# neeharperi/FutureDet

Measured on AMD Instinct MI355X. Metric: sweeps/sec end-to-end (300k pts, 10-sweep voxel), higher is better.
Workload: dtype f32

## Files before the change

futuredet_amd/csrc/fd_common.h:

```cpp
#pragma once
#include <hip/hip_runtime.h>
#include <stdint.h>
#include <stdio.h>

#include <atomic>

#include "../../include/futuredet_hip.h"

namespace fd {

void set_error(const char *fmt, ...);
int spconv_f32_compact_dispatch(const float *in, const void *wp, const float *bias, const float *residual, int relu, const int *nbr,
                                int64_t nbr_stride, int K, int64_t n_in_bound, int n_out, const int *n_out_dev, int cin, int cout, float *out,
                                const int *ranges, int n_ranges, hipStream_t stream);

size_t spconv_bf16_win_weight_bytes(int K, int cin, int cout);
void spconv_bf16_win_pack(const float *w, int K, int cin, int cout, uint16_t (*tobf)(float), uint16_t *dst);
int spconv_bf16_win_dispatch(const void *in, const void *wp_win, const float *bias, const void *residual, int relu, const int *nbr, int64_t nbr_stride, int K,
                             int64_t n_in_bound, int n_out, const int *n_out_dev, int64_t n_expected, int cin, int cout, void *out, hipStream_t stream);
int spconv_bf16_ws_dispatch(const void *in, const void *wp, const float *bias, const void *residual, int relu, const int *nbr, int64_t nbr_stride, int K,
                            int64_t n_in_bound, int n_out, const int *n_out_dev, int64_t n_expected, int cin, int cout, void *out, hipStream_t stream);

int wino_pc_launch(const float *x, const void *wp, const float *bias, float *y, int B, int H, int W, int cin, int cout, int relu, int cout_total,
                   int co_off, hipStream_t stream);

int spconv_f32_res16_dispatch(const float *in, const void *wp, const float *bias, const float *residual, int relu, const int *nbr, int64_t nbr_stride, int K,
                              int64_t n_in_bound, int n_out, const int *n_out_dev, int64_t n_expected, int cin, int cout, float *out, hipStream_t stream);

int spconv_f32_c32_dispatch(const float *in, const void *wp, const float *bias, const float *residual, int relu, const int *nbr,
                            int64_t nbr_stride, int K, int64_t n_in_bound, int n_out, const int *n_out_dev, int cin, int cout, float *out,
                            const int *ranges, int n_ranges, hipStream_t stream);

__device__ __forceinline__ int device_count(int capacity, const int *count_dev) {
    if (!count_dev) return capacity;
    const int n = *count_dev;
    return n < capacity ? (n > 0 ? n : 0) : capacity;
}

inline int check_launch(const char *what) {
    hipError_t e = hipGetLastError();
    if (e != hipSuccess) {
        set_error("%s: %s", what, hipGetErrorString(e));
        return FD_ELAUNCH;
    }
    return FD_OK;
}

#define FD_REQUIRE(cond, ...)           \
    do {                                \
        if (!(cond)) {                  \
            fd::set_error(__VA_ARGS__); \
            return FD_EINVAL;           \
        }                               \
    } while (0)

inline hipStream_t as_stream(fd_stream_t s) { return reinterpret_cast<hipStream_t>(s); }

int fill_words(void *p, uint32_t value, size_t n_words, hipStream_t stream);
int fill_words3(void *p0, uint32_t v0, size_t n0, void *p1, uint32_t v1, size_t n1, void *p2, uint32_t v2, size_t n2, hipStream_t stream);

constexpr int kMaxDevices = 64;
int current_device();
int device_cu_count();
bool ensure_dynamic_lds(const void *kernel, size_t bytes, std::atomic<uint64_t> &done);
enum TuneKey { kTuneSpconvRG = 0, kTuneSpconvV1, kTuneSpconvBf16V1, kTuneV2Depth, kTuneV2TM, kTuneV2LdsPad, kTuneConvNT, kTuneV2RangesPerCU, kTuneV2Uniform, kTuneV2RowCost, kTuneSpconvC32, kTuneBf16GP, kTuneBf16RG, kTuneBf16Depth, kTuneBf16NW, kTuneStrict, kTuneBf16Win, kTuneF32ResRG, kTuneConvStrip, kTuneF32ResNW, kTuneCount };
int tuning(TuneKey key);

inline size_t align_up(size_t v, size_t a) { return (v + a - 1) / a * a; }

struct IndexGeom {
    int B, D, H, W, Ht, Wt;
    __host__ __device__ int64_t num_cols() const { return (int64_t)B * Ht * Wt * 64; }
};
__host__ __device__ inline IndexGeom make_geom(int B, int D, int H, int W) {
    IndexGeom g;
    g.B = B; g.D = D; g.H = H; g.W = W;
    g.Ht = (H + 7) >> 3; g.Wt = (W + 7) >> 3;
    return g;
}
__host__ __device__ inline int64_t col_of(const IndexGeom &g, int b, int y, int x) {
    return ((((int64_t)b * g.Ht + (y >> 3)) * g.Wt + (x >> 3)) << 6) + ((y & 7) << 3) + (x & 7);
}
__device__ inline void col_to_byx(const IndexGeom &g, int64_t col, int &b, int &y, int &x) {
    int in = (int)(col & 63);
    int64_t t = col >> 6;
    int tx = (int)(t % g.Wt);
    t /= g.Wt;
    int ty = (int)(t % g.Ht);
    b = (int)(t / g.Ht);
    y = ty * 8 + (in >> 3);
    x = tx * 8 + (in & 7);
}

__device__ inline unsigned xcd_swizzle(unsigned bid, unsigned nblocks) {
    const unsigned nx = 8;
    unsigned per = nblocks / nx, rem = nblocks % nx;
    unsigned xcd = bid % nx, loc = bid / nx;
    unsigned start = xcd * per + (xcd < rem ? xcd : rem);
    return start + loc;
}

}
```

futuredet_amd/csrc/fd_conv2d_wino.hip:

```cpp
#include "fd_common.h"

#ifndef FD_WINO_OCC16
#define FD_WINO_OCC16 3
#endif

namespace {

#ifdef FD_V2_TRACE
__device__ unsigned long long *g_wtrace;
#define FD_WT(var) const unsigned long long var = __builtin_readcyclecounter()
#define FD_WDECL unsigned long long wacc[8] = {0, 0, 0, 0, 0, 0, 0, 0}
#define FD_WADD(i, v) wacc[i] += (v)
#define FD_WFLUSH                                                                                              \
    do {                                                                                                       \
        if (threadIdx.x == 0 && g_wtrace)                                                                      \
            for (int i_ = 0; i_ < 8; ++i_) g_wtrace[(size_t)(blockIdx.x + blockIdx.y * gridDim.x) * 8 + i_] = wacc[i_]; \
    } while (0)
#else
#define FD_WT(var)
#define FD_WDECL
#define FD_WADD(i, v)
#define FD_WFLUSH
#endif

typedef float f32x4 __attribute__((ext_vector_type(4)));

struct WinoParams {
    int B, H, W, Cin, Cout_pad, Cout_real, cout_total, co_off, relu;
    int tiles_x, tiles_y;
};

__device__ __forceinline__ float4 f4add(float4 a, float4 b) { return make_float4(a.x + b.x, a.y + b.y, a.z + b.z, a.w + b.w); }
__device__ __forceinline__ float4 f4sub(float4 a, float4 b) { return make_float4(a.x - b.x, a.y - b.y, a.z - b.z, a.w - b.w); }

template <int TY, int TX, int NBW>
__global__ void __launch_bounds__(256, (TY * TX * NBW <= 16) ? FD_WINO_OCC16 : (TY * TX * NBW <= 32) ? 2 : 1) conv2d_wino_f32(const float *__restrict__ x, const float4 *__restrict__ wp, const float *__restrict__ bias,
                                                       float *__restrict__ y, WinoParams p) {
    constexpr int NTILE = TY * TX, NTB = NTILE / 16;
    static_assert(NTILE % 16 == 0, "tiles per workgroup must fill whole MFMA blocks");
    constexpr int PH = 2 * TY + 2, PW = 2 * TX + 2, PP = PH * PW;
    constexpr int NCHUNK = PP * 4, NLOAD = (NCHUNK + 255) / 256;
    constexpr int NT = 64 * NBW;
    constexpr int RAW_BYTES = PP * 64, V_BYTES = 16 * NTILE * 64;
    extern __shared__ __attribute__((aligned(16))) unsigned char smem[];
    unsigned char *s_raw = smem, *s_v = smem + RAW_BYTES;

    FD_WDECL;
    FD_WT(tstart);
    const int tid = threadIdx.x, lane = tid & 63, wave = __builtin_amdgcn_readfirstlane(tid >> 6);
    const int lm = lane & 15, lq = lane >> 4;
    int t = blockIdx.x;
    const int tx = t % p.tiles_x; t /= p.tiles_x;
    const int ty = t % p.tiles_y; const int b = t / p.tiles_y;
    const int n0 = blockIdx.y * NT + wave * NBW * 16;
    const int oy0 = ty * 2 * TY, ox0 = tx * 2 * TX;
    const int nslices = p.Cin / 16;

    float4 stage[NLOAD];
    auto load_slice = [&](int s) {
#pragma unroll
        for (int i = 0; i < NLOAD; ++i) {
            const int id = tid + i * 256;
            stage[i] = make_float4(0.f, 0.f, 0.f, 0.f);
            if (id < NCHUNK) {
                const int pix = id >> 2, q = id & 3;
                const int iy = oy0 - 1 + pix / PW, ix = ox0 - 1 + pix % PW;
                if (iy >= 0 && iy < p.H && ix >= 0 && ix < p.W)
                    stage[i] = *reinterpret_cast<const float4 *>(x + (((int64_t)b * p.H + iy) * p.W + ix) * p.Cin + s * 16 + q * 4);
            }
        }
    };
    auto store_raw = [&]() {
#pragma unroll
        for (int i = 0; i < NLOAD; ++i) {
            const int id = tid + i * 256;
            if (id < NCHUNK) *reinterpret_cast<float4 *>(s_raw + id * 16) = stage[i];
        }
    };
    auto transform = [&]() {
        for (int w = tid; w < NTILE * 4 * 2; w += 256) {
            const int half = w & 1, q = (w >> 1) & 3, tile = w >> 3;
            const int py = (tile / TX) * 2, px = (tile % TX) * 2;
            const unsigned char *src = s_raw + ((py + half) * PW + px) * 64 + q * 16;
            float4 d[3][4];
#pragma unroll
            for (int r = 0; r < 3; ++r)
#pragma unroll
                for (int c = 0; c < 4; ++c) d[r][c] = *reinterpret_cast<const float4 *>(src + (r * PW + c) * 64);
            float4 ta[4], tb[4];
#pragma unroll
            for (int c = 0; c < 4; ++c) {
                if (half == 0) { ta[c] = f4sub(d[0][c], d[2][c]); tb[c] = f4add(d[1][c], d[2][c]); }
                else { ta[c] = f4sub(d[1][c], d[0][c]); tb[c] = f4sub(d[0][c], d[2][c]); }
            }
            unsigned char *dst = s_v + (size_t)tile * 64 + q * 16;
            auto put = [&](int row, const float4(&tr)[4]) {
                const float4 v0 = f4sub(tr[0], tr[2]), v1 = f4add(tr[1], tr[2]), v2 = f4sub(tr[2], tr[1]), v3 = f4sub(tr[1], tr[3]);
                *reinterpret_cast<float4 *>(dst + (size_t)(row * 4 + 0) * NTILE * 64) = v0;
                *reinterpret_cast<float4 *>(dst + (size_t)(row * 4 + 1) * NTILE * 64) = v1;
                *reinterpret_cast<float4 *>(dst + (size_t)(row * 4 + 2) * NTILE * 64) = v2;
                *reinterpret_cast<float4 *>(dst + (size_t)(row * 4 + 3) * NTILE * 64) = v3;
            };
            put(half * 2, ta);
            put(half * 2 + 1, tb);
        }
    };

    f32x4 acc[16][NTB][NBW];
#pragma unroll
    for (int xi = 0; xi < 16; ++xi)
#pragma unroll
        for (int i = 0; i < NTB; ++i)
#pragma unroll
            for (int j = 0; j < NBW; ++j) acc[xi][i][j] = f32x4{0.f, 0.f, 0.f, 0.f};

    const int64_t w_nb_stride = (int64_t)nslices * 16 * 64;
    const float4 *wb[NBW];
#pragma unroll
    for (int j = 0; j < NBW; ++j) {
        const int nb = (n0 >> 4) + j;
        wb[j] = wp + (int64_t)(nb < (p.Cout_pad >> 4) ? nb : (p.Cout_pad >> 4) - 1) * w_nb_stride + lane;
    }
    const int total_steps = nslices * 16;
    const unsigned vbase = (unsigned)(lm * 64 + lq * 16);

    load_slice(0);
    constexpr int RW = (NTB * NBW >= 4) ? 2 : 4;
    float4 bw[RW][NBW];
#pragma unroll
    for (int r = 0; r < RW; ++r)
#pragma unroll
        for (int j = 0; j < NBW; ++j) bw[r][j] = wb[j][(int64_t)(r < total_steps ? r : 0) * 64];
    FD_WT(tk0);
    for (int s = 0; s < nslices; ++s) {
        FD_WT(t0);
        store_raw();
        __syncthreads();
        FD_WT(t1);
        if (s + 1 < nslices) load_slice(s + 1);
        transform();
        FD_WT(t2);
        __syncthreads();
        FD_WT(t3);
        float4 a[2][NTB];
#pragma unroll
        for (int i = 0; i < NTB; ++i) a[0][i] = *reinterpret_cast<const float4 *>(s_v + vbase + i * 16 * 64);
#pragma unroll
        for (int xi = 0; xi < 16; ++xi) {
            const int step = s * 16 + xi;
            if (xi + 1 < 16) {
#pragma unroll
                for (int i = 0; i < NTB; ++i)
                    a[(xi + 1) & 1][i] = *reinterpret_cast<const float4 *>(s_v + vbase + ((xi + 1) * NTILE + i * 16) * 64);
            }
            __builtin_amdgcn_sched_barrier(0);
#define FD_KSTEP(C)                                                                                                   \
    _Pragma("unroll") for (int i = 0; i < NTB; ++i) _Pragma("unroll") for (int j = 0; j < NBW; ++j)                   \
        acc[xi][i][j] = __builtin_amdgcn_mfma_f32_16x16x4f32(bw[xi % RW][j].C, a[xi & 1][i].C, acc[xi][i][j], 0, 0, 0);
            FD_KSTEP(x) FD_KSTEP(y) FD_KSTEP(z) FD_KSTEP(w)
#undef FD_KSTEP
            __builtin_amdgcn_sched_barrier(0);
            {
                const int ns = step + RW < total_steps ? step + RW : 0;
#pragma unroll
                for (int j = 0; j < NBW; ++j) bw[xi % RW][j] = wb[j][(int64_t)ns * 64];
            }
        }
        FD_WT(t4);
        __syncthreads();
        FD_WT(t5);
        FD_WADD(0, t1 - t0); FD_WADD(1, t2 - t1); FD_WADD(2, t3 - t2); FD_WADD(3, t4 - t3); FD_WADD(4, t5 - t4);
    }
    FD_WT(tk1);
    FD_WADD(5, ((unsigned long long)__builtin_amdgcn_s_getreg(4 | (31 << 11)) << 32) | (unsigned long long)__builtin_amdgcn_s_getreg(20 | (31 << 11)));
    FD_WADD(6, tstart);
    const bool wide = ((p.cout_total | p.co_off) & 3) == 0;
#pragma unroll
    for (int j = 0; j < NBW; ++j) {
        const int co = n0 + j * 16 + lq * 4;
        float4 bv = make_float4(0.f, 0.f, 0.f, 0.f);
        if (bias && co < p.Cout_real) {
            bv.x = bias[co];
            if (co + 1 < p.Cout_real) bv.y = bias[co + 1];
            if (co + 2 < p.Cout_real) bv.z = bias[co + 2];
            if (co + 3 < p.Cout_real) bv.w = bias[co + 3];
        }
#pragma unroll
        for (int i = 0; i < NTB; ++i) {
            const int tile = i * 16 + lm;
            const int oy = oy0 + (tile / TX) * 2, ox = ox0 + (tile % TX) * 2;
            f32x4 r0[4], r1[4];
#pragma unroll
            for (int c = 0; c < 4; ++c) {
                r0[c] = acc[c][i][j] + acc[4 + c][i][j] + acc[8 + c][i][j];
                r1[c] = acc[4 + c][i][j] - acc[8 + c][i][j] - acc[12 + c][i][j];
            }
            f32x4 yv[2][2];
            yv[0][0] = r0[0] + r0[1] + r0[2];
            yv[0][1] = r0[1] - r0[2] - r0[3];
            yv[1][0] = r1[0] + r1[1] + r1[2];
            yv[1][1] = r1[1] - r1[2] - r1[3];
            if (co >= p.Cout_real) continue;
#pragma unroll
            for (int dy = 0; dy < 2; ++dy)
#pragma unroll
                for (int dx = 0; dx < 2; ++dx) {
                    if (oy + dy >= p.H || ox + dx >= p.W) continue;
                    float4 v = make_float4(yv[dy][dx][0] + bv.x, yv[dy][dx][1] + bv.y, yv[dy][dx][2] + bv.z, yv[dy][dx][3] + bv.w);
                    if (p.relu) { v.x = fmaxf(v.x, 0.f); v.y = fmaxf(v.y, 0.f); v.z = fmaxf(v.z, 0.f); v.w = fmaxf(v.w, 0.f); }
                    float *dst = y + (((int64_t)b * p.H + oy + dy) * p.W + ox + dx) * p.cout_total + p.co_off + co;
                    if (wide && co + 3 < p.Cout_real) {
                        *reinterpret_cast<float4 *>(dst) = v;
                    } else {
                        dst[0] = v.x;
                        if (co + 1 < p.Cout_real) dst[1] = v.y;
                        if (co + 2 < p.Cout_real) dst[2] = v.z;
                        if (co + 3 < p.Cout_real) dst[3] = v.w;
                    }
                }
        }
    }
    FD_WT(tend);
    FD_WADD(7, tend);
    FD_WFLUSH;
}

template <int TY, int TX, int NBW>
bool launch_wino(const float *x, const void *wp, const float *bias, float *y, WinoParams p, hipStream_t stream) {
    constexpr int PH = 2 * TY + 2, PW = 2 * TX + 2;
    const size_t lds = (size_t)PH * PW * 64 + (size_t)16 * TY * TX * 64;
    p.tiles_x = (p.W + 2 * TX - 1) / (2 * TX);
    p.tiles_y = (p.H + 2 * TY - 1) / (2 * TY);
    auto kern = conv2d_wino_f32<TY, TX, NBW>;
    static std::atomic<uint64_t> lds_set{0};
    if (lds > 65536 && !fd::ensure_dynamic_lds(reinterpret_cast<const void *>(kern), lds, lds_set)) return false;
    dim3 grid((unsigned)(p.tiles_x * p.tiles_y * p.B), (unsigned)((p.Cout_real + 64 * NBW - 1) / (64 * NBW)));
    hipLaunchKernelGGL(kern, grid, dim3(256), lds, stream, x, (const float4 *)wp, bias, y, p);
    return true;
}

constexpr int kNumWinoTiles = 7;

}

#ifdef FD_V2_TRACE
extern "C" int fd_debug_set_wino_trace(void *p) { return hipMemcpyToSymbol(HIP_SYMBOL(g_wtrace), &p, sizeof(p)) == hipSuccess ? 0 : -1; }
#endif

extern "C" int fd_conv2d_wino_f32_num_tiles(void) { return kNumWinoTiles; }

extern "C" size_t fd_conv2d_wino_f32_packed_weight_bytes(int cout, int cin) {
    if (cout <= 0 || cin <= 0 || cin % 16) return 0;
    return ((size_t)cout + 63) / 64 * 64 * cin * 16 * 4;
}

extern "C" int fd_conv2d_wino_f32_pack_weight(const float *w, int cout, int cin, void *dst) {
    FD_REQUIRE(w && dst, "fd_conv2d_wino_f32_pack_weight: null argument");
    FD_REQUIRE(cin % 16 == 0 && cout > 0, "fd_conv2d_wino_f32_pack_weight: need cin %% 16 == 0");
    const int cout_pad = (cout + 63) / 64 * 64, nsl = cin / 16;
    static const double G[4][3] = {{1, 0, 0}, {0.5, 0.5, 0.5}, {0.5, -0.5, 0.5}, {0, 0, 1}};
    float *d = (float *)dst;
    for (int nb = 0; nb < cout_pad / 16; ++nb)
        for (int s = 0; s < nsl; ++s)
            for (int lane = 0; lane < 64; ++lane)
                for (int j = 0; j < 4; ++j) {
                    const int co = nb * 16 + (lane & 15), ci = s * 16 + 4 * (lane >> 4) + j;
                    double U[4][4] = {};
                    if (co < cout) {
                        const float *g = w + ((int64_t)co * cin + ci) * 9;
                        double Gg[4][3];
                        for (int r = 0; r < 4; ++r)
                            for (int c = 0; c < 3; ++c) Gg[r][c] = G[r][0] * g[0 * 3 + c] + G[r][1] * g[1 * 3 + c] + G[r][2] * g[2 * 3 + c];
                        for (int r = 0; r < 4; ++r)
                            for (int c = 0; c < 4; ++c) U[r][c] = Gg[r][0] * G[c][0] + Gg[r][1] * G[c][1] + Gg[r][2] * G[c][2];
                    }
                    for (int xi = 0; xi < 16; ++xi)
                        d[((((int64_t)nb * nsl + s) * 16 + xi) * 64 + lane) * 4 + j] = (float)U[xi >> 2][xi & 3];
                }
    return FD_OK;
}

extern "C" int fd_conv2d_wino_nhwc_f32(const float *x, int B, int H, int W, int cin, const void *wpacked, const float *bias, int cout, int relu,
                                       float *y, int cout_total, int co_off, int tile, fd_stream_t stream) {
    FD_REQUIRE(x && wpacked && y, "fd_conv2d_wino_nhwc_f32: null argument");
    FD_REQUIRE(cin % 16 == 0 && cin >= 16, "fd_conv2d_wino_nhwc_f32: cin must be a multiple of 16 (got %d)", cin);
    FD_REQUIRE(B > 0 && H > 0 && W > 0 && cout > 0, "fd_conv2d_wino_nhwc_f32: bad shape");
    FD_REQUIRE(tile >= 0 && tile <= kNumWinoTiles, "fd_conv2d_wino_nhwc_f32: tile must be 0..%d", kNumWinoTiles);
    FD_REQUIRE(co_off >= 0 && co_off + cout <= cout_total, "fd_conv2d_wino_nhwc_f32: channel window [%d, %d) outside the %d output channels", co_off,
               co_off + cout, cout_total);
    WinoParams p;
    p.B = B; p.H = H; p.W = W; p.Cin = cin;
    p.Cout_real = cout;
    p.Cout_pad = (cout + 63) / 64 * 64;
    p.cout_total = cout_total; p.co_off = co_off; p.relu = relu;
    p.tiles_x = p.tiles_y = 0;
    hipStream_t s = fd::as_stream(stream);
    if (tile == 0) tile = 6;
    bool ok;
    switch (tile) {
        case 1: ok = launch_wino<4, 8, 2>(x, wpacked, bias, y, p, s); break;
        case 2: ok = launch_wino<6, 8, 2>(x, wpacked, bias, y, p, s); break;
        case 3: ok = launch_wino<4, 8, 1>(x, wpacked, bias, y, p, s); break;
        case 4: ok = launch_wino<8, 8, 1>(x, wpacked, bias, y, p, s); break;
        case 5: ok = launch_wino<4, 4, 2>(x, wpacked, bias, y, p, s); break;
        case 7: {
            const int rc = fd::wino_pc_launch(x, wpacked, bias, y, B, H, W, cin, cout, relu, cout_total, co_off, s);
            if (rc == 1) {
                fd::set_error("fd_conv2d_wino_nhwc_f32: tile 7 needs W >= 63 and an input below 2 GB (got W = %d)", W);
                return FD_EINVAL;
            }
            ok = rc == 0;
            break;
        }
        default: ok = launch_wino<4, 4, 1>(x, wpacked, bias, y, p, s); break;
    }
    if (!ok) {
        fd::set_error("fd_conv2d_wino_nhwc_f32: the runtime refused tile %d's dynamic LDS request", tile);
        return FD_EINVAL;
    }
    return fd::check_launch("fd_conv2d_wino_nhwc_f32");
}
```

futuredet_amd/csrc/fd_conv2d_wino_pc.hip:

```cpp
#include "fd_common.h"

#include <type_traits>

namespace {

typedef float f32x4 __attribute__((ext_vector_type(4)));

#ifdef FD_V2_TRACE
__device__ unsigned long long *g_pctrace;
#define FD_PT(var) const unsigned long long var = __builtin_readcyclecounter()
#define FD_PADD(i, v) pacc[i] += (v)
#else
#define FD_PT(var)
#define FD_PADD(i, v)
#endif

struct PcParams {
    int B, H, W, Cin, Cout_pad, Cout_real, cout_total, co_off, relu;
    int tiles_x, tiles_y;
    unsigned x_bytes, w_bytes;
    int n_strips, n_items;
};

constexpr int NTB = 2, NTILE = 16 * NTB;
constexpr int XCOLS = 2 * NTILE + 4;
constexpr int N1 = XCOLS * 4;
constexpr int T_ROW = (XCOLS + XCOLS / 4) * 64;
constexpr int T_BYTES = 4 * T_ROW;
constexpr int V_BYTES = 16 * NTILE * 64;
constexpr int kMaxBias = 8192;
constexpr int LDS_BYTES = 2 * T_BYTES + 2 * V_BYTES;
__device__ __forceinline__ int t_off(int x) { return x * 64 + (x >> 2) * 64; }

typedef float f32x2 __attribute__((ext_vector_type(2)));
__device__ __forceinline__ f32x4 sub4(f32x4 a, f32x4 b) {
    f32x2 lo, hi;
    asm("v_pk_add_f32 %0, %1, %2 neg_lo:[0,1] neg_hi:[0,1]" : "=v"(lo) : "v"(__builtin_shufflevector(a, a, 0, 1)), "v"(__builtin_shufflevector(b, b, 0, 1)));
    asm("v_pk_add_f32 %0, %1, %2 neg_lo:[0,1] neg_hi:[0,1]" : "=v"(hi) : "v"(__builtin_shufflevector(a, a, 2, 3)), "v"(__builtin_shufflevector(b, b, 2, 3)));
    return __builtin_shufflevector(lo, hi, 0, 1, 2, 3);
}

__global__ void __launch_bounds__(512) conv2d_wino_pc_f32(const float *__restrict__ x, const float4 *__restrict__ wp, const float *__restrict__ bias,
                                                          float *__restrict__ y, PcParams p) {
    extern __shared__ __attribute__((aligned(16))) unsigned char smem[];
    unsigned char *s_t = smem, *s_v = smem + 2 * T_BYTES;
    float *s_bias = reinterpret_cast<float *>(smem + LDS_BYTES);
    const int tid = threadIdx.x, lane = tid & 63, wave = __builtin_amdgcn_readfirstlane(tid >> 6);
    const int nslices = p.Cin / 16;
    const int tpi = p.tiles_x * p.tiles_y, total = p.B * tpi;
    const int n_mine = (p.n_items - (int)blockIdx.x + (int)gridDim.x - 1) / (int)gridDim.x;
    const int G = n_mine * nslices;

    if (wave >= 4) {
        const int pt = tid - 256;
        const __amdgpu_buffer_rsrc_t xrs = __builtin_amdgcn_make_buffer_rsrc(const_cast<float *>(x), 0, (int)p.x_bytes, 0x00020000);
        const unsigned row_bytes = (unsigned)p.W * (unsigned)p.Cin * 4u;
        unsigned vo0[4], vo1[4];
        constexpr unsigned kOob = 0x80000000u;
        const int xg0 = pt >> 2, xg1 = (pt + 256) >> 2, q = pt & 3;
        auto strip_setup = [&](int item) {
            const int t0 = (item % p.n_strips) * NTILE;
            const int b1 = t0 / tpi, ty1 = (t0 % tpi) / p.tiles_x, tx1 = t0 % p.tiles_x;
            const int n1 = min(NTILE, p.tiles_x - tx1), c1 = 2 * n1 + 2;
            const int t2 = t0 + n1;
            const int n2 = t2 < total ? NTILE - n1 : 0;
            const int b2 = t2 / tpi, ty2 = (t2 % tpi) / p.tiles_x;
            auto one = [&](int xg, bool on, unsigned (&vo)[4]) {
                const bool second = xg >= c1;
                const int xr = second ? xg - c1 : xg;
                const bool live = on && (second ? (n2 > 0 && xr < 2 * n2 + 2) : true);
                const int ix = (second ? 0 : 2 * tx1) - 1 + xr, iy0 = 2 * (second ? ty2 : ty1) - 1;
                const unsigned off = (unsigned)((((int64_t)(second ? b2 : b1) * p.H + iy0) * p.W + ix) * p.Cin + q * 4) * 4u;
#pragma unroll
                for (int r = 0; r < 4; ++r) vo[r] = (live && ix >= 0 && ix < p.W && iy0 + r >= 0 && iy0 + r < p.H) ? off + r * row_bytes : kOob;
            };
            one(xg0, item < p.n_items, vo0);
            one(xg1, item < p.n_items && xg1 < XCOLS, vo1);
        };
        int ld_k = 0, ld_s = 0;
        strip_setup((int)blockIdx.x);
        f32x4 st[2][2][4];
        auto load_step = [&](auto PAR) {
            constexpr int par = decltype(PAR)::value;
#pragma unroll
            for (int r = 0; r < 4; ++r) st[par][0][r] = __builtin_bit_cast(f32x4, __builtin_amdgcn_raw_buffer_load_b128(xrs, vo0[r], ld_s * 64, 0));
#pragma unroll
            for (int r = 0; r < 4; ++r) st[par][1][r] = __builtin_bit_cast(f32x4, __builtin_amdgcn_raw_buffer_load_b128(xrs, vo1[r], ld_s * 64, 0));
            if (++ld_s == nslices) {
                ld_s = 0;
                ++ld_k;
                strip_setup(ld_k < n_mine ? (int)blockIdx.x + ld_k * (int)gridDim.x : p.n_items);
            }
        };
        const int p1o0 = t_off(xg0) + q * 16, p1o1 = t_off(xg1) + q * 16;
        auto pass1_item = [&](const f32x4 (&d)[4], unsigned char *dst) {
            *reinterpret_cast<f32x4 *>(dst + 0 * T_ROW) = sub4(d[0], d[2]);
            *reinterpret_cast<f32x4 *>(dst + 1 * T_ROW) = d[1] + d[2];
            *reinterpret_cast<f32x4 *>(dst + 2 * T_ROW) = sub4(d[2], d[1]);
            *reinterpret_cast<f32x4 *>(dst + 3 * T_ROW) = sub4(d[1], d[3]);
        };
        auto pass1 = [&](auto PAR, unsigned char *t) {
            constexpr int par = decltype(PAR)::value;
            pass1_item(st[par][0], t + p1o0);
            if (wave == 4 && pt < N1 - 256) pass1_item(st[par][1], t + p1o1);
        };
        static_assert(NTILE == 32, "item decoding assumes 32 tiles");
        int p2_left = nslices, p2_k = 0;
        int so[2][2], dof[2];
        auto p2_setup = [&](int item) {
            const int n1 = min(NTILE, p.tiles_x - ((item % p.n_strips) * NTILE) % p.tiles_x);
#pragma unroll
            for (int i = 0; i < 2; ++i) {
                const int w = pt + i * 256;
                const int tile = (w >> 2) & (NTILE - 1), r = w >> 7;
                const int xs = tile < n1 ? 2 * tile : 2 * tile + 2;
                so[i][0] = r * T_ROW + q * 16 + t_off(xs);
                so[i][1] = r * T_ROW + q * 16 + t_off(xs + 2);
                dof[i] = (r * 4) * NTILE * 64 + tile * 64 + q * 16;
            }
        };
        p2_setup((int)blockIdx.x);
        auto pass2 = [&](const unsigned char *t, unsigned char *v) {
#pragma unroll
            for (int i = 0; i < 2; ++i) {
                f32x4 d[4];
                d[0] = *reinterpret_cast<const f32x4 *>(t + so[i][0]);
                d[1] = *reinterpret_cast<const f32x4 *>(t + so[i][0] + 64);
                d[2] = *reinterpret_cast<const f32x4 *>(t + so[i][1]);
                d[3] = *reinterpret_cast<const f32x4 *>(t + so[i][1] + 64);
                unsigned char *dst = v + dof[i];
                *reinterpret_cast<f32x4 *>(dst + 0 * NTILE * 64) = sub4(d[0], d[2]);
                *reinterpret_cast<f32x4 *>(dst + 1 * NTILE * 64) = d[1] + d[2];
                *reinterpret_cast<f32x4 *>(dst + 2 * NTILE * 64) = sub4(d[2], d[1]);
                *reinterpret_cast<f32x4 *>(dst + 3 * NTILE * 64) = sub4(d[1], d[3]);
            }
            if (--p2_left == 0) {
                p2_left = nslices;
                if (++p2_k < n_mine) p2_setup((int)blockIdx.x + p2_k * (int)gridDim.x);
            }
        };
        using P0 = std::integral_constant<int, 0>;
        using P1 = std::integral_constant<int, 1>;
        load_step(P0{});
        load_step(P1{});
        pass1(P0{}, s_t);
        load_step(P0{});
        __syncthreads();
        pass2(s_t, s_v);
        pass1(P1{}, s_t + T_BYTES);
        load_step(P1{});
        __syncthreads();
#ifdef FD_V2_TRACE
        unsigned long long pacc[8] = {0, 0, 0, 0, 0, 0, 0, 0};
#endif
        auto body = [&](auto PAR, int g) {
            constexpr int par = decltype(PAR)::value;
            FD_PT(q0);
            if (g + 1 < G) pass2(s_t + (1 - par) * T_BYTES, s_v + (1 - par) * V_BYTES);
            pass1(PAR, s_t + par * T_BYTES);
            load_step(PAR);
            FD_PT(q1);
            __syncthreads();
            FD_PT(q2);
            FD_PADD(3, q1 - q0); FD_PADD(4, q2 - q1);
        };
        for (int g = 0; g < G; g += 2) {
            body(P0{}, g);
            body(P1{}, g + 1);
        }
#ifdef FD_V2_TRACE
        if (tid == 256 && g_pctrace) { g_pctrace[(size_t)blockIdx.x * 8 + 3] = pacc[3]; g_pctrace[(size_t)blockIdx.x * 8 + 4] = pacc[4]; }
#endif
        return;
    }

#ifdef FD_V2_TRACE
    unsigned long long pacc[8] = {0, 0, 0, 0, 0, 0, 0, 0};
#endif
    FD_PT(tstart);
    const int lm = lane & 15, lq = lane >> 4;
    const unsigned vbase = (unsigned)(lm * 64 + lq * 16);
    const int total_steps = nslices * 16;
    const __amdgpu_buffer_rsrc_t wrs = __builtin_amdgcn_make_buffer_rsrc(const_cast<float4 *>(wp), 0, (int)p.w_bytes, 0x00020000);
    auto weights_of = [&](int item) {
        const int nb = (item / p.n_strips) * 4 + wave;
        return __builtin_amdgcn_readfirstlane((nb < (p.Cout_pad >> 4) ? nb : (p.Cout_pad >> 4) - 1) * total_steps * 1024);
    };
    const unsigned lane16 = lane * 16;
    auto fragment = [&](int base, int step) {
        return __builtin_bit_cast(float4, __builtin_amdgcn_raw_buffer_load_b128(wrs, lane16, base + step * 1024, 0));
    };
    constexpr int RW = 8, AHEAD = 6;
    float4 bw[RW];
    int wb = weights_of((int)blockIdx.x);
#pragma unroll
    for (int r = 0; r < AHEAD; ++r) bw[r] = fragment(wb, r);
    const bool wide = ((p.cout_total | p.co_off) & 3) == 0;
    for (int c = tid; c < p.Cout_pad; c += 256) s_bias[c] = (bias && c < p.Cout_real) ? bias[c] : 0.f;
    __syncthreads();
    __syncthreads();
    FD_PT(tpro);
    FD_PADD(7, tpro - tstart);
    int g = 0;
    for (int k = 0; k < n_mine; ++k) {
        const int item = (int)blockIdx.x + k * (int)gridDim.x;
        const int wnext = k + 1 < n_mine ? weights_of(item + (int)gridDim.x) : wb;
        const int co = (item / p.n_strips) * 64 + wave * 16 + lq * 4;
        f32x4 acc[16][NTB];
#pragma unroll
        for (int xi = 0; xi < 16; ++xi)
#pragma unroll
            for (int i = 0; i < NTB; ++i) acc[xi][i] = f32x4{0.f, 0.f, 0.f, 0.f};
        for (int s = 0; s < nslices; ++s, ++g) {
            const unsigned char *v = s_v + (g & 1) * V_BYTES;
            FD_PT(c0);
            float4 a[2][2][NTB];
#pragma unroll
            for (int e = 0; e < 2; ++e)
#pragma unroll
                for (int i = 0; i < NTB; ++i) a[0][e][i] = *reinterpret_cast<const float4 *>(v + vbase + (e * NTILE + i * 16) * 64);
#pragma unroll
            for (int x2 = 0; x2 < 8; ++x2) {
                const int xi = 2 * x2, step = s * 16 + xi;
#define FD_KSTEP(C)                                                                                                         \
    _Pragma("unroll") for (int e = 0; e < 2; ++e) _Pragma("unroll") for (int i = 0; i < NTB; ++i)                           \
        acc[xi + e][i] = __builtin_amdgcn_mfma_f32_16x16x4f32(bw[(xi + e) % RW].C, a[x2 & 1][e][i].C, acc[xi + e][i], 0, 0, 0);
                __builtin_amdgcn_sched_barrier(0);
                FD_KSTEP(x)
                __builtin_amdgcn_sched_barrier(0);
                if (x2 + 1 < 8) {
#pragma unroll
                    for (int i = 0; i < NTB; ++i) a[(x2 + 1) & 1][0][i] = *reinterpret_cast<const float4 *>(v + vbase + ((xi + 2) * NTILE + i * 16) * 64);
                }
                __builtin_amdgcn_sched_barrier(0);
                FD_KSTEP(y)
                __builtin_amdgcn_sched_barrier(0);
                if (x2 + 1 < 8) {
#pragma unroll
                    for (int i = 0; i < NTB; ++i) a[(x2 + 1) & 1][1][i] = *reinterpret_cast<const float4 *>(v + vbase + ((xi + 3) * NTILE + i * 16) * 64);
                }
                __builtin_amdgcn_sched_barrier(0);
                FD_KSTEP(z)
                __builtin_amdgcn_sched_barrier(0);
#pragma unroll
                for (int e = 0; e < 2; ++e) {
                    const int ns = step + e + AHEAD;
                    bw[(xi + e + AHEAD) % RW] = ns < total_steps ? fragment(wb, ns) : fragment(wnext, ns - total_steps);
                }
                __builtin_amdgcn_sched_barrier(0);
                FD_KSTEP(w)
#undef FD_KSTEP
            }
            __builtin_amdgcn_sched_barrier(0);
            FD_PT(c1);
            __syncthreads();
            FD_PT(c2);
            FD_PADD(0, c1 - c0); FD_PADD(1, c2 - c1);
        }
        wb = wnext;
        FD_PT(e0);

        const int t0 = (item % p.n_strips) * NTILE;
        const int b1 = t0 / tpi, ty1 = (t0 % tpi) / p.tiles_x, tx1 = t0 % p.tiles_x;
        const int n1 = min(NTILE, p.tiles_x - tx1);
        const int t2 = t0 + n1;
        const int n2 = t2 < total ? NTILE - n1 : 0;
        const int b2 = t2 / tpi, ty2 = (t2 % tpi) / p.tiles_x;
        float *const y1 = y + (((int64_t)b1 * p.H + 2 * ty1) * p.W + 2 * tx1) * p.cout_total + p.co_off;
        float *const y2 = y + (((int64_t)b2 * p.H + 2 * ty2) * p.W) * p.cout_total + p.co_off;
        const float4 bv = *reinterpret_cast<const float4 *>(s_bias + co);
        const bool interior = wide && n1 + n2 == NTILE && !((p.H | p.W) & 1) && (item / p.n_strips) * 64 + 64 <= p.Cout_real;
#pragma unroll
        for (int i = 0; i < NTB; ++i) {
            const int j = i * 16 + lm;
            const bool first = j < n1;
            const int jj = first ? j : j - n1;
            const int oy = 2 * (first ? ty1 : ty2), ox = 2 * (first ? tx1 + jj : jj);
            const bool live = (first || jj < n2) && co < p.Cout_real;
            float *const yb = (first ? y1 : y2) + 2 * jj * p.cout_total + co;
            f32x4 r0[4], r1[4];
#pragma unroll
            for (int c = 0; c < 4; ++c) {
                r0[c] = acc[c][i] + acc[4 + c][i] + acc[8 + c][i];
                r1[c] = sub4(sub4(acc[4 + c][i], acc[8 + c][i]), acc[12 + c][i]);
            }
            f32x4 yv[2][2];
            yv[0][0] = r0[0] + r0[1] + r0[2];
            yv[0][1] = sub4(sub4(r0[1], r0[2]), r0[3]);
            yv[1][0] = r1[0] + r1[1] + r1[2];
            yv[1][1] = sub4(sub4(r1[1], r1[2]), r1[3]);
            if (interior) {
#pragma unroll
                for (int dy = 0; dy < 2; ++dy)
#pragma unroll
                    for (int dx = 0; dx < 2; ++dx) {
                        f32x4 v = yv[dy][dx] + f32x4{bv.x, bv.y, bv.z, bv.w};
                        if (p.relu) { v[0] = fmaxf(v[0], 0.f); v[1] = fmaxf(v[1], 0.f); v[2] = fmaxf(v[2], 0.f); v[3] = fmaxf(v[3], 0.f); }
                        *reinterpret_cast<f32x4 *>(yb + (dy * p.W + dx) * p.cout_total) = v;
                    }
                continue;
            }
            if (!live) continue;
#pragma unroll
            for (int dy = 0; dy < 2; ++dy)
#pragma unroll
                for (int dx = 0; dx < 2; ++dx) {
                    if (oy + dy >= p.H || ox + dx >= p.W) continue;
                    float4 v = make_float4(yv[dy][dx][0] + bv.x, yv[dy][dx][1] + bv.y, yv[dy][dx][2] + bv.z, yv[dy][dx][3] + bv.w);
                    if (p.relu) { v.x = fmaxf(v.x, 0.f); v.y = fmaxf(v.y, 0.f); v.z = fmaxf(v.z, 0.f); v.w = fmaxf(v.w, 0.f); }
                    float *dst = yb + (dy * p.W + dx) * p.cout_total;
                    if (wide && co + 3 < p.Cout_real) {
                        *reinterpret_cast<float4 *>(dst) = v;
                    } else {
                        dst[0] = v.x;
                        if (co + 1 < p.Cout_real) dst[1] = v.y;
                        if (co + 2 < p.Cout_real) dst[2] = v.z;
                        if (co + 3 < p.Cout_real) dst[3] = v.w;
                    }
                }
        }
        FD_PT(e1);
        FD_PADD(2, e1 - e0);
    }
    if (G & 1) __syncthreads();
#ifdef FD_V2_TRACE
    if (tid == 0 && g_pctrace) {
        unsigned long long *o = g_pctrace + (size_t)blockIdx.x * 8;
        o[0] = pacc[0]; o[1] = pacc[1]; o[2] = pacc[2]; o[5] = tstart; o[6] = __builtin_readcyclecounter(); o[7] = pacc[7];
    }
#endif
}

}

#ifdef FD_V2_TRACE
extern "C" int fd_debug_set_wino_pc_trace(void *p) { return hipMemcpyToSymbol(HIP_SYMBOL(g_pctrace), &p, sizeof(p)) == hipSuccess ? 0 : -1; }
#endif

namespace fd {

int wino_pc_launch(const float *x, const void *wp, const float *bias, float *y, int B, int H, int W, int cin, int cout, int relu, int cout_total,
                   int co_off, hipStream_t stream) {
    PcParams p;
    p.B = B; p.H = H; p.W = W; p.Cin = cin;
    p.Cout_real = cout;
    p.Cout_pad = (cout + 63) / 64 * 64;
    p.cout_total = cout_total; p.co_off = co_off; p.relu = relu;
    p.tiles_x = (W + 1) / 2;
    p.tiles_y = (H + 1) / 2;
    const int64_t xb = (int64_t)B * H * W * cin * 4;
    const int64_t wbytes = (int64_t)p.Cout_pad * cin * 16 * 4;
    if (p.tiles_x < NTILE || xb >= 0x80000000ll || wbytes >= 0x80000000ll || p.Cout_pad > kMaxBias) return 1;
    p.x_bytes = (unsigned)xb;
    p.w_bytes = (unsigned)wbytes;
    static std::atomic<uint64_t> lds_set{0};
    const size_t lds = (size_t)LDS_BYTES + (size_t)p.Cout_pad * 4;
    if (!fd::ensure_dynamic_lds(reinterpret_cast<const void *>(conv2d_wino_pc_f32), (size_t)LDS_BYTES + kMaxBias * 4, lds_set)) return -1;
    const int64_t n_strips = ((int64_t)p.tiles_x * p.tiles_y * B + NTILE - 1) / NTILE, n_items = n_strips * ((cout + 63) / 64);
    if (n_items >= (1ll << 31)) return 1;
    p.n_strips = (int)n_strips;
    p.n_items = (int)n_items;
    const int n_cu = fd::device_cu_count();
    const int rounds = (int)((n_items + n_cu - 1) / n_cu);
    const unsigned grid = (unsigned)((n_items + rounds - 1) / rounds);
    hipLaunchKernelGGL(conv2d_wino_pc_f32, dim3(grid), dim3(512), lds, stream, x, (const float4 *)wp, bias, y, p);
    return 0;
}

}
```

Before: 277.0.

## Add wide-item Winograd pc kernel variant with eight compute waves per block

Templates the persistent Winograd conv kernel on the number of compute waves, adding an 8-wave (128 output channels per item, 768 threads) variant exposed as a new tile option 8. Each transformed input tile in LDS is reused across twice as many output channels, which cuts the input transform and load work per output. The wide variant uses a simpler MFMA loop with a shallower weight prefetch ring to limit register pressure. It runs only if the tile selector picks option 8, and it may lower occupancy or stall on weight loads.

After: 281.8 (median of 6 runs). 1.7% higher.

```diff
diff --git a/futuredet_amd/csrc/fd_common.h b/futuredet_amd/csrc/fd_common.h
--- a/futuredet_amd/csrc/fd_common.h
+++ b/futuredet_amd/csrc/fd_common.h
@@ -22,7 +22,7 @@
                             int64_t n_in_bound, int n_out, const int *n_out_dev, int64_t n_expected, int cin, int cout, void *out, hipStream_t stream);
 
 int wino_pc_launch(const float *x, const void *wp, const float *bias, float *y, int B, int H, int W, int cin, int cout, int relu, int cout_total,
-                   int co_off, hipStream_t stream);
+                   int co_off, int wide_items, hipStream_t stream);
 
 int spconv_f32_res16_dispatch(const float *in, const void *wp, const float *bias, const float *residual, int relu, const int *nbr, int64_t nbr_stride, int K,
                               int64_t n_in_bound, int n_out, const int *n_out_dev, int64_t n_expected, int cin, int cout, float *out, hipStream_t stream);
diff --git a/futuredet_amd/csrc/fd_conv2d_wino.hip b/futuredet_amd/csrc/fd_conv2d_wino.hip
--- a/futuredet_amd/csrc/fd_conv2d_wino.hip
+++ b/futuredet_amd/csrc/fd_conv2d_wino.hip
@@ -239,7 +239,7 @@
     return true;
 }
 
-constexpr int kNumWinoTiles = 7;
+constexpr int kNumWinoTiles = 8;
 
 }
 
@@ -304,7 +304,7 @@
         case 4: ok = launch_wino<8, 8, 1>(x, wpacked, bias, y, p, s); break;
         case 5: ok = launch_wino<4, 4, 2>(x, wpacked, bias, y, p, s); break;
         case 7: {
-            const int rc = fd::wino_pc_launch(x, wpacked, bias, y, B, H, W, cin, cout, relu, cout_total, co_off, s);
+            const int rc = fd::wino_pc_launch(x, wpacked, bias, y, B, H, W, cin, cout, relu, cout_total, co_off, 0, s);
             if (rc == 1) {
                 fd::set_error("fd_conv2d_wino_nhwc_f32: tile 7 needs W >= 63 and an input below 2 GB (got W = %d)", W);
                 return FD_EINVAL;
@@ -312,6 +312,11 @@
             ok = rc == 0;
             break;
         }
+        case 8: {
+            const int rc = fd::wino_pc_launch(x, wpacked, bias, y, B, H, W, cin, cout, relu, cout_total, co_off, 1, s);
+            ok = rc == 1 ? launch_wino<4, 4, 1>(x, wpacked, bias, y, p, s) : rc == 0;
+            break;
+        }
         default: ok = launch_wino<4, 4, 1>(x, wpacked, bias, y, p, s); break;
     }
     if (!ok) {
diff --git a/futuredet_amd/csrc/fd_conv2d_wino_pc.hip b/futuredet_amd/csrc/fd_conv2d_wino_pc.hip
--- a/futuredet_amd/csrc/fd_conv2d_wino_pc.hip
+++ b/futuredet_amd/csrc/fd_conv2d_wino_pc.hip
@@ -20,6 +20,7 @@
     int tiles_x, tiles_y;
     unsigned x_bytes, w_bytes;
     int n_strips, n_items;
+    int nb_packed;
 };
 
 constexpr int NTB = 2, NTILE = 16 * NTB;
@@ -40,8 +41,10 @@
     return __builtin_shufflevector(lo, hi, 0, 1, 2, 3);
 }
 
-__global__ void __launch_bounds__(512) conv2d_wino_pc_f32(const float *__restrict__ x, const float4 *__restrict__ wp, const float *__restrict__ bias,
-                                                          float *__restrict__ y, PcParams p) {
+template <int NCW>
+__global__ void __launch_bounds__(64 * (NCW + 4)) conv2d_wino_pc_f32(const float *__restrict__ x, const float4 *__restrict__ wp, const float *__restrict__ bias,
+                                                                   float *__restrict__ y, PcParams p) {
+    constexpr int NCT = 64 * NCW, CB = 16 * NCW;
     extern __shared__ __attribute__((aligned(16))) unsigned char smem[];
     unsigned char *s_t = smem, *s_v = smem + 2 * T_BYTES;
     float *s_bias = reinterpret_cast<float *>(smem + LDS_BYTES);
@@ -51,8 +54,8 @@
     const int n_mine = (p.n_items - (int)blockIdx.x + (int)gridDim.x - 1) / (int)gridDim.x;
     const int G = n_mine * nslices;
 
-    if (wave >= 4) {
-        const int pt = tid - 256;
+    if (wave >= NCW) {
+        const int pt = tid - NCT;
         const __amdgpu_buffer_rsrc_t xrs = __builtin_amdgcn_make_buffer_rsrc(const_cast<float *>(x), 0, (int)p.x_bytes, 0x00020000);
         const unsigned row_bytes = (unsigned)p.W * (unsigned)p.Cin * 4u;
         unsigned vo0[4], vo1[4];
@@ -102,7 +105,7 @@
         auto pass1 = [&](auto PAR, unsigned char *t) {
             constexpr int par = decltype(PAR)::value;
             pass1_item(st[par][0], t + p1o0);
-            if (wave == 4 && pt < N1 - 256) pass1_item(st[par][1], t + p1o1);
+            if (wave == NCW && pt < N1 - 256) pass1_item(st[par][1], t + p1o1);
         };
         static_assert(NTILE == 32, "item decoding assumes 32 tiles");
         int p2_left = nslices, p2_k = 0;
@@ -169,7 +172,7 @@
             body(P1{}, g + 1);
         }
 #ifdef FD_V2_TRACE
-        if (tid == 256 && g_pctrace) { g_pctrace[(size_t)blockIdx.x * 8 + 3] = pacc[3]; g_pctrace[(size_t)blockIdx.x * 8 + 4] = pacc[4]; }
+        if (tid == NCT && g_pctrace) { g_pctrace[(size_t)blockIdx.x * 8 + 3] = pacc[3]; g_pctrace[(size_t)blockIdx.x * 8 + 4] = pacc[4]; }
 #endif
         return;
     }
@@ -183,20 +186,20 @@
     const int total_steps = nslices * 16;
     const __amdgpu_buffer_rsrc_t wrs = __builtin_amdgcn_make_buffer_rsrc(const_cast<float4 *>(wp), 0, (int)p.w_bytes, 0x00020000);
     auto weights_of = [&](int item) {
-        const int nb = (item / p.n_strips) * 4 + wave;
-        return __builtin_amdgcn_readfirstlane((nb < (p.Cout_pad >> 4) ? nb : (p.Cout_pad >> 4) - 1) * total_steps * 1024);
+        const int nb = (item / p.n_strips) * NCW + wave;
+        return __builtin_amdgcn_readfirstlane((nb < p.nb_packed ? nb : p.nb_packed - 1) * total_steps * 1024);
     };
     const unsigned lane16 = lane * 16;
     auto fragment = [&](int base, int step) {
         return __builtin_bit_cast(float4, __builtin_amdgcn_raw_buffer_load_b128(wrs, lane16, base + step * 1024, 0));
     };
-    constexpr int RW = 8, AHEAD = 6;
+    constexpr int RW = NCW == 4 ? 8 : 4, AHEAD = NCW == 4 ? 6 : 3;
     float4 bw[RW];
     int wb = weights_of((int)blockIdx.x);
 #pragma unroll
     for (int r = 0; r < AHEAD; ++r) bw[r] = fragment(wb, r);
     const bool wide = ((p.cout_total | p.co_off) & 3) == 0;
-    for (int c = tid; c < p.Cout_pad; c += 256) s_bias[c] = (bias && c < p.Cout_real) ? bias[c] : 0.f;
+    for (int c = tid; c < p.Cout_pad; c += NCT) s_bias[c] = (bias && c < p.Cout_real) ? bias[c] : 0.f;
     __syncthreads();
     __syncthreads();
     FD_PT(tpro);
@@ -205,7 +208,7 @@
     for (int k = 0; k < n_mine; ++k) {
         const int item = (int)blockIdx.x + k * (int)gridDim.x;
         const int wnext = k + 1 < n_mine ? weights_of(item + (int)gridDim.x) : wb;
-        const int co = (item / p.n_strips) * 64 + wave * 16 + lq * 4;
+        const int co = (item / p.n_strips) * CB + wave * 16 + lq * 4;
         f32x4 acc[16][NTB];
 #pragma unroll
         for (int xi = 0; xi < 16; ++xi)
@@ -214,6 +217,7 @@
         for (int s = 0; s < nslices; ++s, ++g) {
             const unsigned char *v = s_v + (g & 1) * V_BYTES;
             FD_PT(c0);
+            if constexpr (NCW == 4) {
             float4 a[2][2][NTB];
 #pragma unroll
             for (int e = 0; e < 2; ++e)
@@ -250,6 +254,29 @@
                 __builtin_amdgcn_sched_barrier(0);
                 FD_KSTEP(w)
 #undef FD_KSTEP
+            }
+            } else {
+            float4 a[NTB];
+#pragma unroll
+            for (int i = 0; i < NTB; ++i) a[i] = *reinterpret_cast<const float4 *>(v + vbase + i * 16 * 64);
+#pragma unroll
+            for (int xi = 0; xi < 16; ++xi) {
+                const int step = s * 16 + xi;
+                {
+                    const int ns = step + AHEAD;
+                    bw[(xi + AHEAD) % RW] = ns < total_steps ? fragment(wb, ns) : fragment(wnext, ns - total_steps);
+                }
+#pragma unroll
+                for (int i = 0; i < NTB; ++i) {
+                    __builtin_amdgcn_sched_barrier(0);
+                    acc[xi][i] = __builtin_amdgcn_mfma_f32_16x16x4f32(bw[xi % RW].x, a[i].x, acc[xi][i], 0, 0, 0);
+                    acc[xi][i] = __builtin_amdgcn_mfma_f32_16x16x4f32(bw[xi % RW].y, a[i].y, acc[xi][i], 0, 0, 0);
+                    acc[xi][i] = __builtin_amdgcn_mfma_f32_16x16x4f32(bw[xi % RW].z, a[i].z, acc[xi][i], 0, 0, 0);
+                    acc[xi][i] = __builtin_amdgcn_mfma_f32_16x16x4f32(bw[xi % RW].w, a[i].w, acc[xi][i], 0, 0, 0);
+                    __builtin_amdgcn_sched_barrier(0);
+                    if (xi + 1 < 16) a[i] = *reinterpret_cast<const float4 *>(v + vbase + ((xi + 1) * NTILE + i * 16) * 64);
+                }
+            }
             }
             __builtin_amdgcn_sched_barrier(0);
             FD_PT(c1);
@@ -269,7 +296,7 @@
         float *const y1 = y + (((int64_t)b1 * p.H + 2 * ty1) * p.W + 2 * tx1) * p.cout_total + p.co_off;
         float *const y2 = y + (((int64_t)b2 * p.H + 2 * ty2) * p.W) * p.cout_total + p.co_off;
         const float4 bv = *reinterpret_cast<const float4 *>(s_bias + co);
-        const bool interior = wide && n1 + n2 == NTILE && !((p.H | p.W) & 1) && (item / p.n_strips) * 64 + 64 <= p.Cout_real;
+        const bool interior = wide && n1 + n2 == NTILE && !((p.H | p.W) & 1) && (item / p.n_strips) * CB + CB <= p.Cout_real;
 #pragma unroll
         for (int i = 0; i < NTB; ++i) {
             const int j = i * 16 + lm;
@@ -340,30 +367,34 @@
 namespace fd {
 
 int wino_pc_launch(const float *x, const void *wp, const float *bias, float *y, int B, int H, int W, int cin, int cout, int relu, int cout_total,
-                   int co_off, hipStream_t stream) {
+                   int co_off, int wide_items, hipStream_t stream) {
+    const int cb = wide_items ? 128 : 64;
     PcParams p;
     p.B = B; p.H = H; p.W = W; p.Cin = cin;
     p.Cout_real = cout;
-    p.Cout_pad = (cout + 63) / 64 * 64;
+    p.Cout_pad = (cout + cb - 1) / cb * cb;
+    p.nb_packed = (cout + 63) / 64 * 4;
     p.cout_total = cout_total; p.co_off = co_off; p.relu = relu;
     p.tiles_x = (W + 1) / 2;
     p.tiles_y = (H + 1) / 2;
     const int64_t xb = (int64_t)B * H * W * cin * 4;
-    const int64_t wbytes = (int64_t)p.Cout_pad * cin * 16 * 4;
+    const int64_t wbytes = (int64_t)p.nb_packed * 16 * cin * 16 * 4;
     if (p.tiles_x < NTILE || xb >= 0x80000000ll || wbytes >= 0x80000000ll || p.Cout_pad > kMaxBias) return 1;
     p.x_bytes = (unsigned)xb;
     p.w_bytes = (unsigned)wbytes;
-    static std::atomic<uint64_t> lds_set{0};
+    static std::atomic<uint64_t> lds_set4{0}, lds_set8{0};
     const size_t lds = (size_t)LDS_BYTES + (size_t)p.Cout_pad * 4;
-    if (!fd::ensure_dynamic_lds(reinterpret_cast<const void *>(conv2d_wino_pc_f32), (size_t)LDS_BYTES + kMaxBias * 4, lds_set)) return -1;
-    const int64_t n_strips = ((int64_t)p.tiles_x * p.tiles_y * B + NTILE - 1) / NTILE, n_items = n_strips * ((cout + 63) / 64);
+    const void *kern = wide_items ? reinterpret_cast<const void *>(conv2d_wino_pc_f32<8>) : reinterpret_cast<const void *>(conv2d_wino_pc_f32<4>);
+    if (!fd::ensure_dynamic_lds(kern, (size_t)LDS_BYTES + kMaxBias * 4, wide_items ? lds_set8 : lds_set4)) return -1;
+    const int64_t n_strips = ((int64_t)p.tiles_x * p.tiles_y * B + NTILE - 1) / NTILE, n_items = n_strips * ((cout + cb - 1) / cb);
     if (n_items >= (1ll << 31)) return 1;
     p.n_strips = (int)n_strips;
     p.n_items = (int)n_items;
     const int n_cu = fd::device_cu_count();
     const int rounds = (int)((n_items + n_cu - 1) / n_cu);
     const unsigned grid = (unsigned)((n_items + rounds - 1) / rounds);
-    hipLaunchKernelGGL(conv2d_wino_pc_f32, dim3(grid), dim3(512), lds, stream, x, (const float4 *)wp, bias, y, p);
+    if (wide_items) hipLaunchKernelGGL(conv2d_wino_pc_f32<8>, dim3(grid), dim3(768), lds, stream, x, (const float4 *)wp, bias, y, p);
+    else hipLaunchKernelGGL(conv2d_wino_pc_f32<4>, dim3(grid), dim3(512), lds, stream, x, (const float4 *)wp, bias, y, p);
     return 0;
 }
 
```
